# muzishen/IMAGDressing

Measured on AMD Instinct MI355X. Metric: 512x512 50-step images/sec (whole node), higher is better.
Workload: dtype bf16

## Files before the change

### imagdressing_amd/csrc/attention.hip

```cpp
#include "common.h"
#include "imd_kernels.h"

namespace {

constexpr int KT = 64;
constexpr int VSTR = KT * 2 + 16;

template <int D> struct AttnCfg {
    static constexpr int DPK = (D + 15) / 16 * 16;
    static constexpr int DPV = (D + 31) / 32 * 32;
    static constexpr int NKT = DPK / 16;
    static constexpr int NDT = DPV / 32;
    static constexpr int KSTR = DPK * 2 + 16;
    static constexpr int VROWS = DPV > D ? D + 1 : DPV;
    static constexpr int VBYTES = VROWS * VSTR;
    static constexpr int BUF = VBYTES + KT * KSTR;
    static_assert((DPV - VROWS) * VSTR <= KT * KSTR, "phantom V^T rows must stay inside the K tile");
    static constexpr int KVECS = (KT * (DPK / 8) + 255) / 256;
    static constexpr int VVECS = (D * (KT / 8) + 255) / 256;
};

typedef __attribute__((__vector_size__(4 * sizeof(uint32_t)))) uint32_t v4u;
__device__ __forceinline__ uint4 buf_load16(const __amdgpu_buffer_rsrc_t& rs, uint32_t byte_off) {
    const v4u v = __builtin_amdgcn_raw_buffer_load_b128(rs, (int)byte_off, 0, 0);
// ... 223 lines not shown
                for (int kb = 0; kb < KB; ++kb)
#pragma unroll
                    for (int r = 0; r < 16; ++r) mx = fmaxf(mx, s[qb][kb][r]);
                mx = fmaxf(mx, __shfl_xor(mx, 32));
                if (OFFS) {
                    if (first || __any(mx > OFFS_THR)) {
                        const float want = m_run[qb] + (first ? mx : fmaxf(mx, 0.f));
                        const float nref = E::tof(E::fromf(want));
                        const float delta = nref - m_run[qb];
                        if (!first) {
                            const float alpha = __builtin_amdgcn_exp2f(-delta);
#pragma unroll
                            for (int dt = 0; dt < C::NDT; ++dt)
#pragma unroll
                                for (int r = 0; r < 16; ++r) o[qb][dt][r] *= alpha;
                        }
#pragma unroll
                        for (int kb = 0; kb < KB; ++kb)
#pragma unroll
                            for (int r = 0; r < 16; ++r) s[qb][kb][r] -= delta;
                        m_run[qb] = nref;
                        if (hi == QPAD_HI) qf[qb][QPAD_T].x = (qf[qb][QPAD_T].x & 0xffff0000u) | (uint32_t)E::fromf(-nref);
                    }
#pragma unroll
                    for (int kb = 0; kb < KB; ++kb)
#pragma unroll
                        for (int r = 0; r < 16; ++r) s[qb][kb][r] = __builtin_amdgcn_exp2f(s[qb][kb][r]);
                } else {
                    const float m_new = fmaxf(m_run[qb], mx);
                    if (__any(m_new != m_run[qb])) {
                        const float alpha = __builtin_amdgcn_exp2f(m_run[qb] - m_new);
                        if (!LSUM_MFMA) l_run[qb] *= alpha;
#pragma unroll
                        for (int dt = 0; dt < C::NDT; ++dt)
#pragma unroll
                            for (int r = 0; r < 16; ++r) o[qb][dt][r] *= alpha;
                        m_run[qb] = m_new;
                    }
                    float psum = 0.f;
#pragma unroll
                    for (int kb = 0; kb < KB; ++kb)
#pragma unroll
                        for (int r = 0; r < 16; ++r) {
                            const float pe = __builtin_amdgcn_exp2f(s[qb][kb][r] - m_new);
                            s[qb][kb][r] = pe;
                            if (!LSUM_MFMA) psum += pe;
                        }
                    if (!LSUM_MFMA) l_run[qb] += psum;
                }
                pack_p();
            };
#pragma unroll
            for (int qb = 0; qb < QW; ++qb) {
                softmax_block(qb);
                if (PVSPLIT) {
#pragma unroll
                    for (int dt = 0; dt < C::NDT; ++dt)
#pragma unroll
                        for (int g = 0; g < 2 * KB; ++g) o[qb][dt] = E::mfma(vfr[dt][g], pf[qb][g], o[qb][dt]);
                        }
            }
            if (!PVSPLIT) {
#pragma unroll
                for (int dt = 0; dt < C::NDT; ++dt)
#pragma unroll
                    for (int g = 0; g < 2 * KB; ++g) {
                        const uint4 vf = *reinterpret_cast<const uint4*>(Vs + dt * 32 * VSTR + vfrag + (2 * k0 + g) * 32);
#pragma unroll
                        for (int qb = 0; qb < QW; ++qb) o[qb][dt] = E::mfma(vf, pf[qb][g], o[qb][dt]);
                    }
            }
            }
            if (t + 1 < ntiles) store_tile((t + 1) & 1);
            __syncthreads();
        }

#pragma unroll
        for (int qb = 0; qb < QW; ++qb) {
            float lt;
            if (LSUM_MFMA) {
                const float mine = o[qb][L_DT][L_REG];
                const float other = __shfl_xor(mine, 32);
                lt = (hi == L_HI) ? mine : other;
            } else {
                lt = l_run[qb] + __shfl_xor(l_run[qb], 32);
            }
            const float inv = ((ph == 1) ? w2 : 1.0f) / lt;
            const int q = q0 + qb * 32 + col;
            if (q >= p.N) continue;
            bf16_t* orow = p.out + ((size_t)b * p.N + q) * p.out_ld + h * D;
#pragma unroll
            for (int dt = 0; dt < C::NDT; ++dt)
#pragma unroll
                for (int j = 0; j < 4; ++j) {
                    const int dd = dt * 32 + 8 * j + 4 * hi;
                    if (dd >= D) continue;
                    float v[4];
#pragma unroll
                    for (int e = 0; e < 4; ++e) v[e] = o[qb][dt][4 * j + e] * inv;
                    if (second_only) {
                        *reinterpret_cast<float4*>(p.phase2_out + ((size_t)b * p.N + q) * (p.H * D) + h * D + dd) = make_float4(v[0], v[1], v[2], v[3]);
                        continue;
                    }
                    if (ph == 1) {
                        const uint2 prev = *reinterpret_cast<const uint2*>(orow + dd);
                        v[0] += E::lo(prev.x); v[1] += E::hi(prev.x); v[2] += E::lo(prev.y); v[3] += E::hi(prev.y);
                    }
                    *reinterpret_cast<uint2*>(orow + dd) = make_uint2(E::pack2(v[0], v[1]), E::pack2(v[2], v[3]));
                }
        }
    }
}

template <bool F16>
__global__ __launch_bounds__(256) void attn_phase_add_kernel(bf16_t* out, int out_ld, const float* __restrict__ add, int C, long rows) {
    using E = El<F16>;
    const int vpr = C / 4;
    const long total = rows * vpr;
    for (long i = blockIdx.x * 256L + threadIdx.x; i < total; i += (long)gridDim.x * 256L) {
        const long r = i / vpr;
        const int c = (int)(i - r * vpr) * 4;
        const float4 a = *reinterpret_cast<const float4*>(add + r * C + c);
        uint2* dst = reinterpret_cast<uint2*>(out + r * out_ld + c);
        const uint2 prev = *dst;
        *dst = make_uint2(E::pack2(a.x + E::lo(prev.x), a.y + E::hi(prev.x)), E::pack2(a.z + E::lo(prev.y), a.w + E::hi(prev.y)));
    }
}

template <bool F16, int D, int QW, int MINW, int KB = 2, bool SPEC = false, int SCHED = 0>
int launch_attn(const AttnParams& p, hipStream_t s) {
    using C = AttnCfg<D>;
    constexpr int lds = 2 * C::BUF;
    auto kern = attn_kernel<F16, D, QW, MINW, KB, SPEC, SCHED>;
    if (int rc_attr = imd_lds_attr(reinterpret_cast<const void*>(kern), lds, "attention")) return rc_attr;
    const int rows = 4 * QW * 32;
    dim3 grid((p.N + rows - 1) / rows, p.H, p.B + (p.phase2_rows > 0 ? p.phase2_rows : 0));
    hipLaunchKernelGGL(kern, grid, dim3(256), lds, s, p);
    int rc = imd_check_launch("attention");
    if (rc || p.phase2_rows <= 0) return rc;
    const long vecs = (long)p.phase2_rows * p.N * (p.H * D / 4);
    const int blocks = (int)((vecs + 255) / 256 < 4096 ? (vecs + 255) / 256 : 4096);
    hipLaunchKernelGGL(attn_phase_add_kernel<F16>, dim3(blocks), dim3(256), 0, s, p.out, p.out_ld, p.phase2_out, p.H * D, (long)p.phase2_rows * p.N);
    return imd_check_launch("attention (phase add)");
}

}

int g_attn_qw40 = 13;

int imd_attn_dpk(int D) { return (D + 15) / 16 * 16; }
int imd_attn_dpv(int D) { return (D + 31) / 32 * 32; }

int g_attn_xcd = 1;
#ifdef IMD_ATTN_SWEEP
int g_attn_v80 = 0, g_attn_v160 = 0;
#endif

int imd_attention_dup_supported(int H, int N, int D) { return (D == 40 && N >= 512 && H > 0) ? 1 : 0; }
int imd_attention_phase_split_supported(int D) { return (D == 64 || D == 80 || D == 160) ? 1 : 0; }

int imd_launch_attention(const AttnParams& p_in, hipStream_t s) {
    AttnParams p = p_in;
    const unsigned tag = (unsigned)p_in.flags & IMD_TUNING_TAG_MASK;
    if (tag != 0 && tag != (unsigned)IMD_TUNING_PER_CALL)
        return imd_set_error("attention: flags = 0x%x on entry is neither 0 nor IMD_TUNING_PER_CALL | bits (an uninitialised parameter block?)", (unsigned)p_in.flags);
    const bool per_call = tag == (unsigned)IMD_TUNING_PER_CALL;
    const int qw40 = (per_call && (p_in.flags & 255)) ? (p_in.flags & 255) : g_attn_qw40;
#ifdef IMD_ABLATIONS
    constexpr int QW40_MAX = 54;
#else
    constexpr int QW40_MAX = 13;
#endif
    if (qw40 < 1 || qw40 > QW40_MAX) return imd_set_error("attention: per-call head-dim-40 variant %d out of range 1..%d", qw40, QW40_MAX);
    p.flags = (per_call ? !((p_in.flags >> 8) & 1) : g_attn_xcd != 0) ? 0 : 1;
    if (p.B <= 0 || p.H <= 0 || p.N <= 0 || p.L1 <= 0) return imd_set_error("attention: empty problem B=%d H=%d N=%d L1=%d", p.B, p.H, p.N, p.L1);
    if (p.L1P % 64 || p.L1P < p.L1) return imd_set_error("attention: L1P (%d) must be a multiple of 64 and >= L1 (%d)", p.L1P, p.L1);
    if (p.k2 && (p.L2 <= 0 || p.L2P % 64 || p.L2P < p.L2)) return imd_set_error("attention: bad second key set L2=%d L2P=%d", p.L2, p.L2P);
    if (p.kv1_bdiv <= 0 || (p.k2 && p.kv2_bdiv <= 0)) return imd_set_error("attention: kv batch divisors must be positive");
    if (p.H > 65535 || p.B > 65535) return imd_set_error("attention: H/B exceed grid limits");
    if (p.dtype != IMD_DTYPE_BF16 && p.dtype != IMD_DTYPE_F16) return imd_set_error("attention: unknown dtype %d", p.dtype);
    if (p.causal && (p.k2 != nullptr || p.L1 != p.N)) return imd_set_error("attention: the causal mask needs a single key set with L1 == N");
    const bool h = p.dtype == IMD_DTYPE_F16;
    if ((p.phase2_rows != 0) != (p.phase2_out != nullptr)) return imd_set_error("attention: phase2_rows and phase2_out go together");
    if (p.phase2_rows != 0) {
        if (!imd_attention_phase_split_supported(p.D) || p.k2 == nullptr || p.scale2 == nullptr || p.causal || p.proj_w != nullptr || p.out_dup != nullptr ||
            p.phase2_rows < 0 || p.phase2_rows > p.B || (p.out_ld % 4) || p.B + p.phase2_rows > 65535)
            return imd_set_error("attention: phase2_rows needs head dim 64 / 80 / 160, a second key set with scale2, 0 < rows <= B, no causal mask / fused out-projection / "
                                 "out_dup (got D=%d rows=%d B=%d)", p.D, p.phase2_rows, p.B);
        if ((reinterpret_cast<uintptr_t>(p.phase2_out) & 15) || (reinterpret_cast<uintptr_t>(p.out) & 7))
            return imd_set_error("attention: phase2_out must be 16-byte aligned (out 8-byte)");
    }
    if (p.out_dup != nullptr) {
        if (!imd_attention_dup_supported(p.H, p.N, p.D) || !p.k_pad_one || p.causal || p.proj_w != nullptr)
            return imd_set_error("attention: out_dup needs head dim 40, N >= 512, k_pad_one, no causal mask and no fused out-projection (got D=%d N=%d k_pad_one=%d)", p.D, p.N, p.k_pad_one);
        if (p.out_dup == p.out) return imd_set_error("attention: out_dup must not alias out");
        return imd_launch_attention_d40(p, qw40 == 12 ? 12 : 13, s);
    }
    if (p.proj_w != nullptr) {
        if (p.D != 40 || p.H * p.D != 320 || p.N < 512 || p.causal)
            return imd_set_error("attention: the fused out-projection needs head dim 40, 8 heads, N >= 512, no causal mask (got D=%d H=%d N=%d)", p.D, p.H, p.N);
        if (!p.proj_out || !p.proj_counters) return imd_set_error("attention: fused out-projection without proj_out / proj_counters");
        if ((p.out_ld % 8) || (p.proj_out_ld % 8) || (p.proj_res && (p.proj_res_ld % 8)))
            return imd_set_error("attention: fused out-projection needs out_ld, proj_out_ld and proj_res_ld %% 8 == 0");
        if ((reinterpret_cast<uintptr_t>(p.out) | reinterpret_cast<uintptr_t>(p.proj_w) | reinterpret_cast<uintptr_t>(p.proj_out) |
             reinterpret_cast<uintptr_t>(p.proj_res) | reinterpret_cast<uintptr_t>(p.proj_b)) & 15)
            return imd_set_error("attention: fused out-projection needs 16-byte aligned out / proj_w / proj_out / proj_res / proj_b");
        if ((size_t)p.B * p.N * p.out_ld * 2 >= 0x80000000ull) return imd_set_error("attention: fused out-projection: out buffer beyond 2 GiB");
        return imd_launch_attention_d40(p, 10, s);
    }
    switch (p.D) {
        case 40:
            if (qw40 >= 6 && p.N >= 512 && !p.causal) return imd_launch_attention_d40(p, qw40, s);
            if (qw40 == 2 && p.N >= 512) return h ? launch_attn<true, 40, 2, 2, 1, true, 1>(p, s) : launch_attn<false, 40, 2, 2, 1, true, 1>(p, s);
            if (qw40 == 5 && p.N >= 512) return h ? launch_attn<true, 40, 2, 2, 1, true, 3>(p, s) : launch_attn<false, 40, 2, 2, 1, true, 3>(p, s);
            if (qw40 == 3) return h ? launch_attn<true, 40, 1, 3, 2, false>(p, s) : launch_attn<false, 40, 1, 3, 2, false>(p, s);
            if (qw40 == 4) return h ? launch_attn<true, 40, 1, 3, 1, true>(p, s) : launch_attn<false, 40, 1, 3, 1, true>(p, s);
            if (qw40 == 1 && p.N >= 512) return h ? launch_attn<true, 40, 2, 2, 1, true, 0>(p, s) : launch_attn<false, 40, 2, 2, 1, true, 0>(p, s);
            return h ? launch_attn<true, 40, 1, 3, 1, true>(p, s) : launch_attn<false, 40, 1, 3, 1, true>(p, s);
        case 64: return h ? launch_attn<true, 64, 1, 2>(p, s) : launch_attn<false, 64, 1, 2>(p, s);
        case 80:
#ifdef IMD_ATTN_SWEEP
            switch (g_attn_v80) {
                case 1: return h ? launch_attn<true, 80, 1, 2, 2, false, 0>(p, s) : launch_attn<false, 80, 1, 2, 2, false, 0>(p, s);
                case 2: return h ? launch_attn<true, 80, 1, 3, 1, false, 0>(p, s) : launch_attn<false, 80, 1, 3, 1, false, 0>(p, s);
                case 3: return h ? launch_attn<true, 80, 1, 3, 1, false, 2>(p, s) : launch_attn<false, 80, 1, 3, 1, false, 2>(p, s);
                case 4: return h ? launch_attn<true, 80, 2, 1, 2, false, 0>(p, s) : launch_attn<false, 80, 2, 1, 2, false, 0>(p, s);
                case 5: return h ? launch_attn<true, 80, 2, 1, 2, false, 3>(p, s) : launch_attn<false, 80, 2, 1, 2, false, 3>(p, s);
                case 6: return h ? launch_attn<true, 80, 2, 1, 1, false, 3>(p, s) : launch_attn<false, 80, 2, 1, 1, false, 3>(p, s);
                case 7: return h ? launch_attn<true, 80, 1, 2, 1, false, 2>(p, s) : launch_attn<false, 80, 1, 2, 1, false, 2>(p, s);
                default: break;
            }
#endif
            return h ? launch_attn<true, 80, 1, 2, 2, false, 2>(p, s) : launch_attn<false, 80, 1, 2, 2, false, 2>(p, s);
        case 160:
#ifdef IMD_ATTN_SWEEP
            switch (g_attn_v160) {
                case 1: return h ? launch_attn<true, 160, 1, 1, 2, false, 0>(p, s) : launch_attn<false, 160, 1, 1, 2, false, 0>(p, s);
                case 2: return h ? launch_attn<true, 160, 1, 1, 1, false, 2>(p, s) : launch_attn<false, 160, 1, 1, 1, false, 2>(p, s);
                case 3: return h ? launch_attn<true, 160, 1, 2, 1, false, 0>(p, s) : launch_attn<false, 160, 1, 2, 1, false, 0>(p, s);
                default: break;
            }
#endif
            return h ? launch_attn<true, 160, 1, 1, 2, false, 2>(p, s) : launch_attn<false, 160, 1, 1, 2, false, 2>(p, s);
        default: return imd_set_error("attention: unsupported head dim %d (supported: 40, 64, 80, 160)", p.D);
    }
}
```

### imagdressing_amd/csrc/capi.cpp

```cpp
#include <atomic>
#include <mutex>
#include <stdarg.h>
#include <stdio.h>
#include <string.h>

#include "imd_kernels.h"

namespace {
thread_local char g_err[512] = "";
}

int imd_set_error(const char* fmt, ...) {
    va_list ap;
    va_start(ap, fmt);
    vsnprintf(g_err, sizeof(g_err), fmt, ap);
    va_end(ap);
    return 1;
}

int imd_check_launch(const char* what) {
    hipError_t e = hipGetLastError();
    if (e != hipSuccess) return imd_set_error("%s: launch failed: %s", what, hipGetErrorString(e));
    return 0;
}

#define IMD_REQUIRE(cond, ...) do { if (!(cond)) return imd_set_error(__VA_ARGS__); } while (0)
#define IMD_REQUIRE_SIZE(p, what) IMD_REQUIRE((p)->struct_bytes == sizeof(*(p)), \
    "%s: parameter block is %u bytes in the caller's view, this library (ABI v%d) expects %zu: the binding mirrors another version of include/imagdressing_hip.h (set struct_bytes = sizeof(struct) after zero-initialising it)", \
    what, (unsigned)(p)->struct_bytes, IMD_ABI_VERSION, sizeof(*(p)))

namespace {
struct LdsAttrEnt { const void* kern; int dev; };
constexpr int kMaxLdsAttr = 512;
LdsAttrEnt g_lds_attr[kMaxLdsAttr];
std::atomic<int> g_lds_attr_n{0};
std::mutex g_lds_attr_mu;
int g_cu8[64] = {};
}

int imd_lds_attr(const void* kern, int bytes, const char* what) {
    int dev = 0;
    if (hipGetDevice(&dev) != hipSuccess) return imd_set_error("%s: cannot identify the current device", what);
    const int n = g_lds_attr_n.load(std::memory_order_acquire);
    for (int i = 0; i < n; ++i)
        if (g_lds_attr[i].kern == kern && g_lds_attr[i].dev == dev) return 0;
    std::lock_guard<std::mutex> lock(g_lds_attr_mu);
    hipError_t e = hipFuncSetAttribute(kern, hipFuncAttributeMaxDynamicSharedMemorySize, bytes);
    if (e != hipSuccess) return imd_set_error("%s: hipFuncSetAttribute failed: %s", what, hipGetErrorString(e));
    const int m = g_lds_attr_n.load(std::memory_order_relaxed);
    if (m < kMaxLdsAttr) {
        g_lds_attr[m] = LdsAttrEnt{kern, dev};
        g_lds_attr_n.store(m + 1, std::memory_order_release);
    }
    return 0;
}

int imd_cu_count8() {
    int dev = 0;
    if (hipGetDevice(&dev) != hipSuccess || dev < 0 || dev >= 64) return -1;
    if (g_cu8[dev] == 0) {
        int cus = 0;
        if (hipDeviceGetAttribute(&cus, hipDeviceAttributeMultiprocessorCount, dev) != hipSuccess) return -1;
        g_cu8[dev] = cus / 8 * 8 < 8 ? 8 : cus / 8 * 8;
    }
    return g_cu8[dev];
}

extern "C" {

int imd_abi_version(void) { return IMD_ABI_VERSION; }
const char* imd_last_error(void) { return g_err; }

int imd_device_check(int device) {
    hipDeviceProp_t prop;
    hipError_t e = hipGetDeviceProperties(&prop, device);
    if (e != hipSuccess) return imd_set_error("device_check: hipGetDeviceProperties(%d) failed: %s", device, hipGetErrorString(e));
    if (strncmp(prop.gcnArchName, "gfx950", 6) != 0)
        return imd_set_error("device_check: device %d is %s; this library is built for gfx950 (MI355X) only", device, prop.gcnArchName);
    return 0;
}

int imd_conv_gemm(const imd_conv_gemm_params* p, int cfg, void* stream) {
    IMD_REQUIRE(p != nullptr, "conv_gemm: null params");
    IMD_REQUIRE_SIZE(p, "conv_gemm");
    IMD_REQUIRE(p->x && p->w, "conv_gemm: null input/weight pointer");
    IMD_REQUIRE(p->mode == IMD_OUT_HEADS || p->out != nullptr, "conv_gemm: null output pointer");
    IMD_REQUIRE(p->Hout > 0 && p->Wout > 0 && p->Hin > 0 && p->Win > 0, "conv_gemm: bad geometry");
    IMD_REQUIRE(p->stride == 1 || p->stride == 2, "conv_gemm: stride must be 1 or 2");
    IMD_REQUIRE(p->M % (p->Hout * p->Wout) == 0, "conv_gemm: M (%d) is not a multiple of Hout*Wout (%d)", p->M, p->Hout * p->Wout);
    if (p->mode == IMD_OUT_HEADS) {
        IMD_REQUIRE(p->hC > 0 && p->hH > 0 && p->hD > 0 && p->hC == p->hH * p->hD, "conv_gemm: bad head split C=%d H=%d D=%d", p->hC, p->hH, p->hD);
        IMD_REQUIRE(p->N % p->hC == 0 && p->N / p->hC <= 3, "conv_gemm: N (%d) must be 1..3 splits of %d channels", p->N, p->hC);
        IMD_REQUIRE(p->hD % 8 == 0, "conv_gemm: head dim must be a multiple of 8");
        IMD_REQUIRE(p->act != IMD_ACT_GEGLU && !p->out_f32, "conv_gemm: head-split output excludes GEGLU / fp32 output");
    }
    if (p->act == IMD_ACT_GEGLU) IMD_REQUIRE(!p->out_f32 && !p->res, "conv_gemm: GEGLU excludes fp32 output and residual");
    return imd_launch_conv_gemm(*p, cfg, (hipStream_t)stream);
}

int imd_conv_gemm_auto_cfg(int M, int N) { return imd_conv_gemm_choose_cfg(M, N); }
int imd_conv_gemm_auto_split(int M, int N, int K, int cfg) { return imd_conv_gemm_choose_split(M, N, K, cfg < 0 ? imd_conv_gemm_choose_cfg(M, N) : cfg); }

int imd_attention(const imd_attn_params* p, void* stream) {
    IMD_REQUIRE(p != nullptr, "attention: null params");
    IMD_REQUIRE_SIZE(p, "attention");
    IMD_REQUIRE(p->q && p->k1 && p->v1t && p->out, "attention: null q/k/v/out pointer");
    IMD_REQUIRE((p->k2 == nullptr) == (p->v2t == nullptr), "attention: k2 and v2t must be given together");
    IMD_REQUIRE(p->out_ld >= p->H * p->D && p->out_ld % 4 == 0, "attention: bad out_ld %d", p->out_ld);
    return imd_launch_attention(*p, (hipStream_t)stream);
}

int imd_attention_fp8(const imd_attn_params* p, int eq, int ek, int ev, void* stream) {
    IMD_REQUIRE(p != nullptr, "attention_fp8: null params");
    IMD_REQUIRE_SIZE(p, "attention_fp8");
    IMD_REQUIRE(p->q && p->k1 && p->v1t && p->out, "attention_fp8: null q/k/v/out pointer");
    IMD_REQUIRE((p->k2 == nullptr) == (p->v2t == nullptr), "attention_fp8: k2 and v2t must be given together");
    IMD_REQUIRE(p->out_ld >= p->H * p->D && p->out_ld % 4 == 0, "attention_fp8: bad out_ld %d", p->out_ld);
    IMD_REQUIRE(p->dtype == IMD_DTYPE_BF16 || p->dtype == IMD_DTYPE_F16, "attention_fp8: unknown output dtype %d", p->dtype);
    return imd_launch_attention_fp8(*p, eq, ek, ev, (hipStream_t)stream);
}

int imd_attn_quantize_fp8(const uint16_t* src, uint8_t* dst, int kind, long count, int LP, int exp2_scale, float pad_val, int dtype,
                          void* stream) {
    IMD_REQUIRE(src && dst && count > 0, "attn_quantize_fp8: null pointer / empty");
    IMD_REQUIRE(kind == 0 || kind == 1, "attn_quantize_fp8: kind must be 0 (Q / K rows) or 1 (V^T)");
    IMD_REQUIRE(exp2_scale >= -16 && exp2_scale <= 16, "attn_quantize_fp8: exponent out of range");
    return imd_launch_attn_quantize_fp8(src, dst, kind, count, LP, exp2_scale, pad_val, dtype, (hipStream_t)stream);
}

int imd_set_tuning(int knob, int value) {
    switch (knob) {
        case 0:
#ifdef IMD_ABLATIONS
            IMD_REQUIRE(value >= 1 && value <= 54, "set_tuning: attention variant for head dim 40 must be 1..54 (20..49: timing ablations, WRONG results; 50..54: correct but no faster)");
#else
            IMD_REQUIRE(value >= 1 && value <= 13, "set_tuning: attention variant for head dim 40 must be 1..13 (the timing ablations 20..49 and the measured no-gain variants 50..54 exist only in -DIMD_ABLATIONS builds)");
#endif
            g_attn_qw40 = value; return 0;
        case 1: g_attn_xcd = value ? 1 : 0; return 0;
        case 2:
#ifndef IMD_ABLATIONS
            IMD_REQUIRE((value & 224) == 0, "set_tuning: bits 5..7 of knob 2 are the timing ablations of gemm_dma256.hip (WRONG results); they exist only in -DIMD_ABLATIONS builds");
#endif
            IMD_REQUIRE((value & ~2047) == 0, "set_tuning: knob 2 has bits 0..10 only (got %d)", value);
            g_gemm_flags = value; return 0;
#ifdef IMD_ATTN_SWEEP
        case 3: g_attn_v80 = value; return 0;
        case 4: g_attn_v160 = value; return 0;
#endif
        default: return imd_set_error("set_tuning: unknown knob %d", knob);
    }
}

int imd_get_tuning(int knob) { return knob == 0 ? g_attn_qw40 : knob == 1 ? g_attn_xcd : knob == 2 ? g_gemm_flags : -1; }

int imd_attn_padded_dims(int D, int* dpk, int* dpv) {
    IMD_REQUIRE(D == 40 || D == 64 || D == 80 || D == 160, "attn_padded_dims: unsupported head dim %d", D);
    if (dpk) *dpk = imd_attn_dpk(D);
    if (dpv) *dpv = imd_attn_dpv(D);
    return 0;
}

int imd_groupnorm(const imd_groupnorm_params* p, void* stream) {
    IMD_REQUIRE(p != nullptr, "groupnorm: null params");
    IMD_REQUIRE_SIZE(p, "groupnorm");
    IMD_REQUIRE(p->x && p->y && p->gamma && p->beta && p->partial, "groupnorm: null pointer");
    return imd_launch_groupnorm(*p, (hipStream_t)stream);
}

int imd_groupnorm_coeffs(const imd_groupnorm_params* p, float* coef_a, float* coef_b, void* stream) {
    IMD_REQUIRE(p != nullptr, "groupnorm_coeffs: null params");
    IMD_REQUIRE_SIZE(p, "groupnorm_coeffs");
    IMD_REQUIRE(p->x && p->gamma && p->beta && p->partial && coef_a && coef_b, "groupnorm_coeffs: null pointer");
    return imd_launch_groupnorm_coeffs(*p, coef_a, coef_b, (hipStream_t)stream);
}

static bool sized(const imd_conv_gemm_params* p) { return p && p->struct_bytes == sizeof(*p); }
static int query(const imd_conv_gemm_params* p, bool (*pred)(const imd_conv_gemm_params&)) {
    if (!sized(p)) return 0;
    imd_conv_gemm_params q = *p;
    if (!imd_conv_gemm_fill_extents(q)) return 0;
    return pred(q) ? 1 : 0;
}
int imd_conv_patch_supported(const imd_conv_gemm_params* p) { return query(p, static_cast<bool (*)(const imd_conv_gemm_params&)>(imd_conv_patch_supported)); }
int imd_conv_patch2_supported(const imd_conv_gemm_params* p) { return query(p, static_cast<bool (*)(const imd_conv_gemm_params&)>(imd_conv_patch2_supported)); }
int imd_conv_patch3_supported(const imd_conv_gemm_params* p) { return query(p, static_cast<bool (*)(const imd_conv_gemm_params&)>(imd_conv_patch3_supported)); }
int imd_conv_patch4_supported(const imd_conv_gemm_params* p) { return query(p, static_cast<bool (*)(const imd_conv_gemm_params&)>(imd_conv_patch4_supported)); }
int imd_conv_img_supported(const imd_conv_gemm_params* p) { return query(p, static_cast<bool (*)(const imd_conv_gemm_params&)>(imd_conv_img_supported)); }
int imd_conv_patch_stats_parts(const imd_conv_gemm_params* p) { return sized(p) ? imd_conv_patch_stats_parts_of(*p) : 0; }
int imd_conv_gemm_stats_parts(const imd_conv_gemm_params* p, int cfg) { return sized(p) ? imd_conv_gemm_stats_parts_of(*p, cfg) : 0; }
int imd_row_linear_gn_in_supported(const imd_conv_gemm_params* p, int cfg) { return (sized(p) && p->gn_in_partial != nullptr && imd_row_linear_gn_in_supported_of(*p, cfg)) ? 1 : 0; }
int imd_conv_gemm_gn_out_supported(const imd_conv_gemm_params* p) { return (sized(p) && imd_conv_gemm_gn_out_supported_of(*p, -1)) ? 1 : 0; }
int imd_gemm_dma_supported(const imd_conv_gemm_params* p) { return query(p, static_cast<bool (*)(const imd_conv_gemm_params&)>(imd_gemm_dma_supported)); }

int imd_row_linear_supported(const imd_conv_gemm_params* p) { return (sized(p) && (imd_row_linear_supported(*p) || imd_row_linear_k640_supported(*p) || imd_row_linear_k1280_supported(*p) || imd_row_qkv_supported(*p))) ? 1 : 0; }

int imd_row_linear(const imd_conv_gemm_params* p, int ln, float ln_eps, void* stream) {
    IMD_REQUIRE(p != nullptr, "row_linear: null params");
    IMD_REQUIRE_SIZE(p, "row_linear");
    IMD_REQUIRE(p->x && p->w, "row_linear: null input/weight pointer");
    IMD_REQUIRE(p->mode == IMD_OUT_HEADS || p->out != nullptr, "row_linear: null output pointer");
    IMD_REQUIRE(p->Hout > 0 && p->Wout > 0 && p->M > 0 && p->M % (p->Hout * p->Wout) == 0, "row_linear: bad geometry");
    if (p->mode == IMD_OUT_HEADS) {
        IMD_REQUIRE(p->hC > 0 && p->hH > 0 && p->hD > 0 && p->hC == p->hH * p->hD && p->N % p->hC == 0 && p->N / p->hC <= 3 && p->hD % 8 == 0,
                    "row_linear: bad head split C=%d H=%d D=%d", p->hC, p->hH, p->hD);
        IMD_REQUIRE(!p->out_f32, "row_linear: head-split output excludes fp32 output");
    }
    IMD_REQUIRE(!ln || ln_eps > 0.f, "row_linear: LayerNorm needs eps > 0");
    if (p->K == 320 && p->N == 960 && p->mode == IMD_OUT_HEADS) {
        IMD_REQUIRE(p->gn_in_partial == nullptr, "row_linear: the fused q / k / v projection has no GroupNorm prologue (gn_in_*)");
        return imd_launch_row_qkv(*p, ln, ln_eps, (hipStream_t)stream);
    }
    if (p->K == 640) return imd_launch_row_linear_k640(*p, ln, ln_eps, (hipStream_t)stream);
    if (p->K == 1280) return imd_launch_row_linear_k1280(*p, ln, ln_eps, (hipStream_t)stream);
    return imd_launch_row_linear(*p, ln, ln_eps, (hipStream_t)stream);
}

int imd_ff_geglu(const imd_ff_params* p, void* stream) {
    IMD_REQUIRE(p != nullptr, "ff_geglu: null params");
    IMD_REQUIRE_SIZE(p, "ff_geglu");
    IMD_REQUIRE(p->x && p->w1 && p->b1 && p->w2 && p->b2 && p->out, "ff_geglu: null pointer");
    IMD_REQUIRE(!p->ln || p->ln_eps > 0.f, "ff_geglu: LayerNorm needs eps > 0");
    return imd_launch_ff_geglu(*p, (hipStream_t)stream);
}

int imd_layernorm(const imd_layernorm_params* p, void* stream) {
    IMD_REQUIRE(p != nullptr, "layernorm: null params");
    IMD_REQUIRE_SIZE(p, "layernorm");
    IMD_REQUIRE(p->x && p->y && p->gamma && p->beta, "layernorm: null pointer");
    return imd_launch_layernorm(*p, (hipStream_t)stream);
}

int imd_embed_tokens(const uint16_t* table, int vocab, const uint16_t* pos, int T, const int64_t* ids, uint16_t* out, long rows, int C,
                     int dtype, void* stream) {
    IMD_REQUIRE(table && pos && ids && out, "embed_tokens: null pointer");
    return imd_launch_embed_tokens(table, vocab, pos, T, ids, out, rows, C, dtype, (hipStream_t)stream);
}

int imd_vit_assemble(const uint16_t* patches, const uint16_t* cls, const uint16_t* pos, uint16_t* out, int B, int P, int C, int dtype,
                     void* stream) {
    IMD_REQUIRE(patches && cls && pos && out, "vit_assemble: null pointer");
    return imd_launch_vit_assemble(patches, cls, pos, out, B, P, C, dtype, (hipStream_t)stream);
}

int imd_lincomb(const float* const* xs, const float* coefs, int n, float* out, long numel, void* stream) {
    IMD_REQUIRE(xs && coefs && out, "lincomb: null pointer");
    return imd_launch_lincomb(xs, coefs, n, out, numel, (hipStream_t)stream);
}

int imd_softmax_rows(const float* s, int s_ld, uint16_t* p, int p_ld, int rows, int cols, int dtype, void* stream) {
    IMD_REQUIRE(s && p, "softmax_rows: null pointer");
    return imd_launch_softmax_rows(s, s_ld, p, p_ld, rows, cols, dtype, (hipStream_t)stream);
}

int imd_ddim_cfg_step(const imd_ddim_params* p, void* stream) {
    IMD_REQUIRE(p != nullptr, "ddim_cfg_step: null params");
    IMD_REQUIRE_SIZE(p, "ddim_cfg_step");
    IMD_REQUIRE(p->z && p->eps, "ddim_cfg_step: null pointer");
    IMD_REQUIRE(p->coefs != nullptr || p->sqrt_a_t > 0.f, "ddim_cfg_step: sqrt(alpha_t) must be positive");
    return imd_launch_ddim_cfg_step(*p, (hipStream_t)stream);
}

int imd_ddim_cfg_step_rows(const imd_ddim_params* p, const float* guidance, void* stream) {
    IMD_REQUIRE(p != nullptr, "ddim_cfg_step_rows: null params");
    IMD_REQUIRE_SIZE(p, "ddim_cfg_step_rows");
    IMD_REQUIRE(p->z && p->eps && guidance, "ddim_cfg_step_rows: null pointer");
    IMD_REQUIRE(p->coefs != nullptr || p->sqrt_a_t > 0.f, "ddim_cfg_step_rows: sqrt(alpha_t) must be positive");
    return imd_launch_ddim_cfg_step_rows(*p, guidance, (hipStream_t)stream);
}

int imd_timestep_embedding(const float* t, float* out, int B, int dim, void* stream) {
    IMD_REQUIRE(t && out, "timestep_embedding: null pointer");
    return imd_launch_timestep_embedding(t, out, B, dim, (hipStream_t)stream);
}

int imd_add(const uint16_t* a, int a_ld, const uint16_t* b, int b_ld, uint16_t* out, int out_ld, long rows, int C, float b_scale, int dtype, void* stream) {
    IMD_REQUIRE(a && b && out, "add: null pointer");
    return imd_launch_add(a, a_ld, b, b_ld, out, out_ld, rows, C, b_scale, dtype, (hipStream_t)stream);
}

int imd_copy2d(const uint16_t* a, int a_ld, uint16_t* out, int out_ld, long rows, int C, void* stream) {
    IMD_REQUIRE(a && out, "copy2d: null pointer");
    return imd_launch_copy2d(a, a_ld, out, out_ld, rows, C, (hipStream_t)stream);
}

int imd_concat2(const uint16_t* a, int Ca, const uint16_t* b, int Cb, const uint16_t* b_add, uint16_t* out, long rows, long b_rows, int dtype, void* stream) {
    IMD_REQUIRE(a && b && out, "concat2: null pointer");
    return imd_launch_concat2(a, Ca, b, Cb, b_add, out, rows, b_rows, dtype, (hipStream_t)stream);
}

int imd_groupnorm_parts(int B, int HW, int C) { return imd_groupnorm_parts_of(B, HW, C); }

int imd_concat2_gn_stats(const uint16_t* a, int Ca, const uint16_t* b, int Cb, const uint16_t* b_add, uint16_t* out, int B, int HW, int b_B, int G,
                         float* partial, int dtype, void* stream) {
    IMD_REQUIRE(a && b && out && partial, "concat2 + statistics: null pointer");
    return imd_launch_concat2_gn_stats(a, Ca, b, Cb, b_add, out, B, HW, b_B, G, partial, dtype, (hipStream_t)stream);
}

int imd_f32_to_16(const float* a, uint16_t* out, long n, int dtype, void* stream) {
    IMD_REQUIRE(a && out, "f32_to_16: null pointer");
// ... 5 lines not shown
```

### imagdressing_amd/csrc/imd_kernels.h

```cpp
#pragma once
#include <hip/hip_runtime.h>
#include <stdint.h>

#include "../../include/imagdressing_hip.h"

typedef uint16_t bf16_t;
typedef imd_heads_dest HeadsDest;
typedef imd_conv_gemm_params ConvGemmParams;
typedef imd_attn_params AttnParams;
typedef imd_groupnorm_params GroupNormParams;
typedef imd_layernorm_params LayerNormParams;
typedef imd_ddim_params DdimParams;

enum { ACT_NONE = IMD_ACT_NONE, ACT_SILU = IMD_ACT_SILU, ACT_GEGLU = IMD_ACT_GEGLU, ACT_GELU = IMD_ACT_GELU, ACT_QUICK_GELU = IMD_ACT_QUICK_GELU };
enum { OUT_ROWMAJOR = IMD_OUT_ROWMAJOR, OUT_HEADS = IMD_OUT_HEADS };

int imd_set_error(const char* fmt, ...);
int imd_check_launch(const char* what);
int imd_lds_attr(const void* kern, int bytes, const char* what);
int imd_cu_count8();

int imd_conv_gemm_choose_cfg(int M, int N);
int imd_conv_gemm_choose_split(int M, int N, int K, int cfg);
int imd_launch_conv_gemm(const ConvGemmParams& p, int cfg, hipStream_t s);
bool imd_conv_gemm_fill_extents(ConvGemmParams& p);
bool imd_conv_patch_supported(const ConvGemmParams& p);
bool imd_conv_patch2_supported(const ConvGemmParams& p);
int imd_launch_conv_patch2(const ConvGemmParams& p, hipStream_t s);
bool imd_conv_patch3_supported(const ConvGemmParams& p);
int imd_launch_conv_patch3(const ConvGemmParams& p, hipStream_t s);
bool imd_conv_patch4_supported(const ConvGemmParams& p);
int imd_launch_conv_patch4(const ConvGemmParams& p, hipStream_t s);
int imd_conv_patch3_stats_parts_of(const ConvGemmParams& p, int nw);
bool imd_conv_patch64_supported(const ConvGemmParams& p);
int imd_launch_conv_patch64(const ConvGemmParams& p, hipStream_t s);
bool imd_conv_img_supported(const ConvGemmParams& p);
int imd_launch_conv_img(const ConvGemmParams& p, hipStream_t s);
int imd_conv_patch_stats_parts_of(const ConvGemmParams& p);
int imd_conv_gemm_stats_parts_of(const ConvGemmParams& p, int cfg);
bool imd_conv_gemm_gn_out_supported_of(const ConvGemmParams& p, int cfg);
bool imd_row_linear_gn_in_supported_of(const ConvGemmParams& p, int cfg);
int imd_launch_conv_patch(const ConvGemmParams& p, hipStream_t s);
bool imd_row_linear_supported(const ConvGemmParams& p);
int imd_launch_row_linear(const ConvGemmParams& p, int ln, float ln_eps, hipStream_t s);
bool imd_row_linear_k640_supported(const ConvGemmParams& p);
int imd_launch_row_linear_k640(const ConvGemmParams& p, int ln, float ln_eps, hipStream_t s);
bool imd_row_linear_k1280_supported(const ConvGemmParams& p);
int imd_launch_row_linear_k1280(const ConvGemmParams& p, int ln, float ln_eps, hipStream_t s);
bool imd_row_qkv_supported(const ConvGemmParams& p);
int imd_launch_row_qkv(const ConvGemmParams& p, int ln, float ln_eps, hipStream_t s);
bool imd_gemm_dma_supported(const ConvGemmParams& p);
int imd_launch_gemm_dma(const ConvGemmParams& p, hipStream_t s);
int imd_launch_gemm_dma128(const ConvGemmParams& p, int stages, hipStream_t s);
int imd_launch_gemm_dma256(const ConvGemmParams& p, int form, hipStream_t s);
bool imd_conv_dma_supported(const ConvGemmParams& p);
int imd_launch_ff_geglu(const imd_ff_params& p, hipStream_t s);
int imd_launch_attention(const AttnParams& p, hipStream_t s);
int imd_launch_attention_d40(const AttnParams& p, int variant, hipStream_t s);
int imd_launch_attention_fp8(const AttnParams& p, int eq, int ek, int ev, hipStream_t s);
int imd_launch_attn_quantize_fp8(const bf16_t* src, unsigned char* dst, int kind, long rows_or_groups, int LP, int exp2_scale,
                                 float pad_val, int dtype, hipStream_t s);
extern int g_attn_qw40;
extern int g_attn_xcd;
#ifdef IMD_ATTN_SWEEP
extern int g_attn_v80, g_attn_v160;
#endif
extern int g_gemm_flags;
int imd_attn_dpk(int D);
int imd_attn_dpv(int D);
int imd_launch_groupnorm(const GroupNormParams& p, hipStream_t s);
int imd_launch_groupnorm_coeffs(const GroupNormParams& p, float* ca, float* cb, hipStream_t s);
int imd_groupnorm_parts_of(int B, int HW, int C);
int imd_launch_concat2_gn_stats(const bf16_t* a, int Ca, const bf16_t* b, int Cb, const bf16_t* b_add, bf16_t* out, int B, int HW, int b_B, int G,
                                float* partial, int dtype, hipStream_t s);
int imd_launch_layernorm(const LayerNormParams& p, hipStream_t s);
int imd_launch_softmax_rows(const float* s_in, int s_ld, bf16_t* p_out, int p_ld, int rows, int cols, int dtype, hipStream_t s);
int imd_launch_ddim_cfg_step(const DdimParams& p, hipStream_t s);
int imd_launch_ddim_cfg_step_rows(const DdimParams& p, const float* guidance, hipStream_t s);
int imd_launch_timestep_embedding(const float* t, float* out, int B, int dim, hipStream_t s);
int imd_launch_add(const bf16_t* a, int a_ld, const bf16_t* b, int b_ld, bf16_t* out, int out_ld, long rows, int C, float b_scale, int dtype, hipStream_t s);
int imd_launch_embed_tokens(const bf16_t* table, int vocab, const bf16_t* pos, int T, const int64_t* ids, bf16_t* out, long rows, int C, int dtype, hipStream_t s);
int imd_launch_vit_assemble(const bf16_t* patches, const bf16_t* cls, const bf16_t* pos, bf16_t* out, int B, int P, int C, int dtype, hipStream_t s);
int imd_launch_lincomb(const float* const* xs, const float* coefs, int n, float* out, long numel, hipStream_t s);
int imd_launch_copy2d(const bf16_t* a, int a_ld, bf16_t* out, int out_ld, long rows, int C, hipStream_t s);
int imd_launch_concat2(const bf16_t* a, int Ca, const bf16_t* b, int Cb, const bf16_t* b_add, bf16_t* out, long rows, long b_rows, int dtype, hipStream_t s);
int imd_launch_f32_to_16(const float* a, bf16_t* out, long n, int dtype, hipStream_t s);
```

Measured before the change: 6.957.

## Add dedicated head-dim-80 attention kernel with LDS DMA ring pipeline

Adds a specialised flash-attention kernel for head dimension 80. It streams K and V^T tiles into a three-slot LDS ring using buffer-to-LDS DMA, and software-pipelines the fragment loads, MFMAs and softmax work across two 32-key steps. It also uses a lazy max-offset rescaling that only rescales when the running max grows past a threshold. The kernel is dispatched by default for non-causal, single-phase calls with N>=512 and L1>128, replacing the generic templated path there. This adds a large new code path with XCD-aware block remapping, at the cost of more complexity and a risk of numerical or edge-case differences.

Measured after the change: 6.978, median of 6. No clear change (+0.3%).

```diff
diff --git a/imagdressing_amd/csrc/attention.hip b/imagdressing_amd/csrc/attention.hip
--- a/imagdressing_amd/csrc/attention.hip
+++ b/imagdressing_amd/csrc/attention.hip
@@ -399,8 +399,10 @@
 int imd_attn_dpv(int D) { return (D + 31) / 32 * 32; }
 
 int g_attn_xcd = 1;
+int g_attn_v80 = 0;
+constexpr int ATTN80_MIN_N = 512, ATTN80_MIN_L1 = 128;
 #ifdef IMD_ATTN_SWEEP
-int g_attn_v80 = 0, g_attn_v160 = 0;
+int g_attn_v160 = 0;
 #endif
 
 int imd_attention_dup_supported(int H, int N, int D) { return (D == 40 && N >= 512 && H > 0) ? 1 : 0; }
@@ -466,10 +468,18 @@
             return h ? launch_attn<true, 40, 1, 3, 1, true>(p, s) : launch_attn<false, 40, 1, 3, 1, true>(p, s);
         case 64: return h ? launch_attn<true, 64, 1, 2>(p, s) : launch_attn<false, 64, 1, 2>(p, s);
         case 80:
+            if (!p.causal && p.phase2_rows == 0 && (g_attn_v80 == 2 || (p.N >= ATTN80_MIN_N && p.L1 > ATTN80_MIN_L1))) {
+                if (g_attn_v80 == 0 || g_attn_v80 == 2) return imd_launch_attention_d80(p, 0, s);
+#ifdef IMD_ATTN_SWEEP
+                if (g_attn_v80 == 9) return imd_launch_attention_d80(p, 9, s);
+#endif
+#ifdef IMD_ABLATIONS
+                if (g_attn_v80 >= 20) return imd_launch_attention_d80(p, g_attn_v80, s);
+#endif
+            }
 #ifdef IMD_ATTN_SWEEP
             switch (g_attn_v80) {
                 case 1: return h ? launch_attn<true, 80, 1, 2, 2, false, 0>(p, s) : launch_attn<false, 80, 1, 2, 2, false, 0>(p, s);
-                case 2: return h ? launch_attn<true, 80, 1, 3, 1, false, 0>(p, s) : launch_attn<false, 80, 1, 3, 1, false, 0>(p, s);
                 case 3: return h ? launch_attn<true, 80, 1, 3, 1, false, 2>(p, s) : launch_attn<false, 80, 1, 3, 1, false, 2>(p, s);
                 case 4: return h ? launch_attn<true, 80, 2, 1, 2, false, 0>(p, s) : launch_attn<false, 80, 2, 1, 2, false, 0>(p, s);
                 case 5: return h ? launch_attn<true, 80, 2, 1, 2, false, 3>(p, s) : launch_attn<false, 80, 2, 1, 2, false, 3>(p, s);
diff --git a/imagdressing_amd/csrc/attention_d80.hip b/imagdressing_amd/csrc/attention_d80.hip
--- /dev/null
+++ b/imagdressing_amd/csrc/attention_d80.hip
@@ -0,0 +1,323 @@
+#include <type_traits>
+#include "lds_dma.h"
+
+#include "common.h"
+#include "imd_kernels.h"
+
+namespace {
+
+constexpr int D = 80, DPK = 80, DPV = 96, NKT = DPK / 16, NDT = DPV / 32;
+constexpr int KT = 64;
+constexpr int KSTR = DPK * 2, VSTR = KT * 2;
+constexpr int VROWS = D + 1;
+constexpr int VBYTES = VROWS * VSTR;
+constexpr int KBYTES = KT * KSTR;
+constexpr int BUF = VBYTES + KBYTES;
+static_assert((DPV - VROWS) * VSTR <= KBYTES, "phantom V^T rows must stay inside the K rows");
+constexpr int NRING = 3;
+constexpr int NKP = KBYTES / 1024, NVP = D * VSTR / 1024, NPIECE = (NKP + NVP) / 4;
+static_assert(NKP * 1024 == KBYTES && NVP * 1024 == D * VSTR && NPIECE * 4 == NKP + NVP, "a unit is a whole number of pieces per wave");
+constexpr int NF = NKT + 2 * NDT;
+constexpr uint32_t OOB = 0xffffffffu;
+constexpr int QW_SHIP = 1;
+
+template <bool F16, int QW, int VAR>
+__global__ __launch_bounds__(256, QW == 1 ? 2 : 1) void attn80_kernel(const AttnParams p) {
+    using E = El<F16>;
+    constexpr int L_DT = D / 32, L_REG = ((D % 32) & 3) + 4 * ((D % 32) >> 3), L_HI = ((D % 32) >> 2) & 1;
+    constexpr int PD = QW == 1 ? 3 : 2;
+    constexpr int NFR = PD + 1;
+    constexpr int NM = NF * QW;
+    constexpr float OFFS_THR = 8.0f;
+    extern __shared__ __attribute__((aligned(16))) char smem[];
+
+    const int tid = threadIdx.x;
+    const int lane = tid & 63;
+    const int wave = tid >> 6;
+    const int hi = lane >> 5;
+    const int col = lane & 31;
+    int wx, h, b;
+    {
+        const unsigned gx = gridDim.x, gy = gridDim.y, gz = gridDim.z, total = gx * gy * gz;
+        const unsigned Lb = blockIdx.x + gx * (blockIdx.y + gy * blockIdx.z);
+        const unsigned xcd = Lb & 7u, slot = Lb >> 3;
+        const unsigned q8 = total >> 3, r8 = total & 7u;
+        unsigned w = (xcd < r8 ? xcd * (q8 + 1) : r8 * (q8 + 1) + (xcd - r8) * q8) + slot;
+        if (p.flags & 1) w = Lb;
+        wx = (int)(w % gx);
+        b = (int)((w / gx) % gz);
+        h = (int)(w / (gx * gz));
+    }
+    const int q0 = (wx * 4 + wave) * (QW * 32);
+
+    {
+        const uint32_t one2 = E::pack2(1.0f, 1.0f);
+        for (int v = tid; v < NRING * (VSTR / 16); v += 256)
+            *reinterpret_cast<uint4*>(smem + (v / (VSTR / 16)) * BUF + D * VSTR + (v % (VSTR / 16)) * 16) = make_uint4(one2, one2, one2, one2);
+    }
+
+    uint4 qf[QW][NKT];
+#pragma unroll
+    for (int qb = 0; qb < QW; ++qb) {
+        const int q = q0 + qb * 32 + col;
+#pragma unroll
+        for (int t = 0; t < NKT; ++t) {
+            uint4 v = make_uint4(0, 0, 0, 0);
+            if (q < p.N) v = *reinterpret_cast<const uint4*>(p.q + ((size_t)(b * p.H + h) * p.N + q) * DPK + t * 16 + hi * 8);
+            qf[qb][t] = v;
+        }
+    }
+
+    float w2 = 0.f;
+    if (p.k2 != nullptr && p.scale2 != nullptr) w2 = p.scale2[b];
+    const int nph = (w2 != 0.f) ? 2 : 1;
+
+    const int kfd = swap23(col) * KSTR + ((hi ^ ((col >> 2) & 1)) << 4);
+    int vfd[4];
+#pragma unroll
+    for (int g = 0; g < 4; ++g) vfd[g] = col * VSTR + (((2 * g + hi) ^ ((col >> 1) & 7)) << 4);
+    const f32x16 zero16 = {0.f, 0.f, 0.f, 0.f, 0.f, 0.f, 0.f, 0.f, 0.f, 0.f, 0.f, 0.f, 0.f, 0.f, 0.f, 0.f};
+    const int wv = __builtin_amdgcn_readfirstlane(wave);
+    const uint32_t smem_base = (uint32_t)(uintptr_t)smem;
+
+    for (int ph = 0; ph < nph; ++ph) {
+        f32x16 o[QW][NDT];
+        float m_ref[QW];
+        f32x16 cinit[QW];
+#pragma unroll
+        for (int qb = 0; qb < QW; ++qb) {
+            m_ref[qb] = 0.f;
+            cinit[qb] = zero16;
+#pragma unroll
+            for (int dt = 0; dt < NDT; ++dt) o[qb][dt] = zero16;
+        }
+        const int L = ph ? p.L2 : p.L1;
+        const int LP = ph ? p.L2P : p.L1P;
+        const int kvb = ph ? (b / p.kv2_bdiv) : (b / p.kv1_bdiv);
+        const bf16_t* kbase = (ph ? p.k2 : p.k1) + (size_t)(kvb * p.H + h) * L * DPK;
+        const bf16_t* vbase = (ph ? p.v2t : p.v1t) + (size_t)(kvb * p.H + h) * DPV * LP;
+        const int J = (L + 31) >> 5;
+        const int NU = (J >> 1) + 1;
+
+        const v4i_t ds_k = raw_rsrc(kbase, (uint32_t)L * DPK * 2), ds_v = raw_rsrc(vbase, (uint32_t)D * LP * 2);
+        int dsrc[NPIECE];
+        bool dneg[NPIECE];
+#pragma unroll
+        for (int i = 0; i < NPIECE; ++i) {
+            const int qi = wv + 4 * i;
+            if (qi < NKP) {
+                const int sl = 64 * qi + lane, r = sl / 10, c = (sl % 10) ^ ((r >> 3) & 1);
+                dsrc[i] = (32 + r) * KSTR + c * 16;
+                dneg[i] = r < 32;
+            } else {
+                const int sl = 64 * (qi - NKP) + lane, dd = sl >> 3, c = (sl & 7) ^ ((dd >> 1) & 7);
+                dsrc[i] = (dd * LP + c * 8 - 32) * 2;
+                dneg[i] = c < 4;
+            }
+        }
+        auto dma_piece = [&](int u, int bufi, int i, auto loop_c) __attribute__((always_inline)) {
+            constexpr bool LOOP = decltype(loop_c)::value;
+            const int qi = wv + 4 * i;
+            const bool isk = qi < NKP;
+            const bool bad = !LOOP && (isk ? (u < 0 && dneg[i]) : (u <= 0 && (u < 0 || dneg[i])));
+            const uint32_t off = bad ? OOB : (uint32_t)(dsrc[i] + u * (isk ? KBYTES : KT * 2));
+            const uint32_t dst = smem_base + bufi * BUF + (isk ? VBYTES + 1024 * qi : 1024 * (qi - NKP));
+            if (LOOP) dma16_nonop(isk ? ds_k : ds_v, dst, off);
+            else dma16(isk ? ds_k : ds_v, dst, off);
+        };
+        auto dma_unit = [&](int u, int bufi, auto loop_c) __attribute__((always_inline)) {
+#pragma unroll
+            for (int i = 0; i < NPIECE; ++i) dma_piece(u, bufi, i, loop_c);
+        };
+
+        f32x16 sa[QW], sb[QW];
+        uint4 pa[QW][2], pb[QW][2];
+#pragma unroll
+        for (int qb = 0; qb < QW; ++qb)
+#pragma unroll
+            for (int g = 0; g < 2; ++g) pb[qb][g] = make_uint4(0, 0, 0, 0);
+        uint4 fr[NFR];
+
+        auto step = [&](const char* Vs, auto second_c, int j, f32x16 (&sc)[QW], f32x16 (&sn)[QW], uint4 (&pc)[QW][2], uint4 (&pp)[QW][2]) __attribute__((always_inline)) {
+            constexpr bool SECOND = decltype(second_c)::value;
+            constexpr int KB = SECOND ? 1 : 0, G0 = SECOND ? 2 : 0, R0 = SECOND ? (NF % NFR) : 0;
+            const char* Ks = Vs + VBYTES;
+            if (j * 32 + 32 > L) {
+#pragma unroll
+                for (int qb = 0; qb < QW; ++qb)
+#pragma unroll
+                    for (int r = 0; r < 16; ++r) {
+                        const int key = j * 32 + 8 * hi + (r & 7) + 16 * (r >> 3);
+                        if (key >= L) sc[qb][r] = -INFINITY;
+                    }
+            }
+            auto frag = [&](int f, int kb, int g0) -> uint4 {
+                if ((VAR & 1024) && f > 0) f = 0;
+                return f < NKT ? *reinterpret_cast<const uint4*>(Ks + kb * 32 * KSTR + kfd + f * 32)
+                               : *reinterpret_cast<const uint4*>(Vs + ((f - NKT) >> 1) * 32 * VSTR + vfd[g0 + ((f - NKT) & 1)]);
+            };
+            auto mma = [&](int i, const uint4& fa) {
+                const int f = i / QW, qb = i % QW;
+                if (f < NKT) { if (!(VAR & 64) || f == 0) sn[qb] = E::mfma(fa, qf[qb][f], f == 0 ? cinit[qb] : sn[qb]); }
+                else if (!(VAR & 32)) o[qb][(f - NKT) >> 1] = E::mfma(fa, pp[qb][(f - NKT) & 1], o[qb][(f - NKT) >> 1]);
+            };
+            float dlt[QW];
+#pragma unroll
+            for (int qb = 0; qb < QW; ++qb) dlt[qb] = 0.f;
+            bool fix = false;
+            auto word = [&](int qb, int w) -> uint32_t& {
+                uint4& v = pc[qb][w >> 2];
+                return (w & 3) == 0 ? v.x : (w & 3) == 1 ? v.y : (w & 3) == 2 ? v.z : v.w;
+            };
+            auto vwork = [&](int qb, int k) {
+                if (k == 0) {
+                    float mx = __builtin_fmaxf(__builtin_fmaxf(sc[qb][0], sc[qb][1]), sc[qb][2]);
+#pragma unroll
+                    for (int r = 3; r < 15; r += 2) mx = __builtin_fmaxf(__builtin_fmaxf(mx, sc[qb][r]), sc[qb][r + 1]);
+                    mx = __builtin_fmaxf(mx, sc[qb][15]);
+                    const auto sw = __builtin_amdgcn_permlane32_swap(__float_as_uint(mx), __float_as_uint(mx), false, false);
+                    mx = __builtin_fmaxf(__uint_as_float(sw[0]), __uint_as_float(sw[1]));
+                    const bool first = j == 0;
+                    if (__builtin_expect(first || __any(mx > OFFS_THR), 0)) {
+                        const float d = first ? mx : __builtin_fmaxf(mx, 0.f);
+#pragma unroll
+                        for (int r = 0; r < 16; ++r) sc[qb][r] -= d;
+                        m_ref[qb] += d;
+#pragma unroll
+                        for (int r = 0; r < 16; ++r) cinit[qb][r] = -m_ref[qb];
+                        dlt[qb] = d;
+                        fix = true;
+                    }
+                    return;
+                }
+                if (k <= 8 && !(VAR & 4)) {
+                    const int r0 = 2 * (k - 1);
+                    sc[qb][r0] = __builtin_amdgcn_exp2f(sc[qb][r0]);
+                    sc[qb][r0 + 1] = __builtin_amdgcn_exp2f(sc[qb][r0 + 1]);
+                }
+                if (k >= 2 && k <= 9) {
+                    uint32_t& w = word(qb, k - 2);
+                    w = E::pack2(sc[qb][2 * (k - 2)], sc[qb][2 * (k - 2) + 1]);
+                    asm volatile("" : "+v"(w));
+                }
+            };
+            if (!SECOND) {
+#pragma unroll
+                for (int f = 0; f < PD; ++f) fr[f] = frag(f, KB, G0);
+            }
+            __builtin_amdgcn_sched_barrier(0);
+#pragma unroll
+            for (int i = 0; i < NM; ++i) {
+                if (i % QW == 0) {
+                    const int f2 = i / QW + PD;
+                    if (f2 < NF) fr[(R0 + f2) % NFR] = frag(f2, KB, G0);
+                    else if (!SECOND) fr[(R0 + f2) % NFR] = frag(f2 - NF, 1, 2);
+                }
+                mma(i, fr[(R0 + i / QW) % NFR]);
+                vwork(i / NF, i % NF);
+                __builtin_amdgcn_sched_barrier(0);
+            }
+            if (fix) {
+#pragma unroll
+                for (int qb = 0; qb < QW; ++qb) {
+#pragma unroll
+                    for (int r = 0; r < 16; ++r) sn[qb][r] -= dlt[qb];
+                    if (j != 0) {
+                        const float alpha = __builtin_amdgcn_exp2f(-dlt[qb]);
+#pragma unroll
+                        for (int dt = 0; dt < NDT; ++dt)
+#pragma unroll
+                            for (int r = 0; r < 16; ++r) o[qb][dt][r] *= alpha;
+                    }
+                }
+            }
+        };
+
+        dma_unit(-1, 2, std::false_type{});
+        dma_unit(0, 0, std::false_type{});
+        dma_unit(1, 1, std::false_type{});
+        dma_wait();
+        __syncthreads();
+        {
+            const char* Ks = smem + 2 * BUF + VBYTES + 32 * KSTR;
+#pragma unroll
+            for (int tk = 0; tk < NKT; ++tk) {
+                const uint4 kf = *reinterpret_cast<const uint4*>(Ks + kfd + tk * 32);
+#pragma unroll
+                for (int qb = 0; qb < QW; ++qb) sa[qb] = E::mfma(kf, qf[qb][tk], tk == 0 ? zero16 : sa[qb]);
+            }
+        }
+        __syncthreads();
+
+        int ring = 0;
+        for (int u = 0; u < NU; ++u) {
+            const int dbuf = ring == 0 ? 2 : ring - 1;
+            if (!(VAR & 16)) dma_unit(u + 2, dbuf, std::true_type{});
+            const char* Vs = smem + ring * BUF;
+            ring = ring == NRING - 1 ? 0 : ring + 1;
+            step(Vs, std::false_type{}, 2 * u, sa, sb, pa, pb);
+            step(Vs, std::true_type{}, 2 * u + 1, sb, sa, pb, pa);
+            dma_wait_keep_n<NPIECE>();
+            if (!(VAR & 8)) __syncthreads();
+        }
+        dma_wait();
+        __syncthreads();
+
+#pragma unroll
+        for (int qb = 0; qb < QW; ++qb) {
+            const float mine = o[qb][L_DT][L_REG];
+            const float other = __shfl_xor(mine, 32);
+            const float lt = (hi == L_HI) ? mine : other;
+            const float inv = ((ph == 1) ? w2 : 1.0f) / lt;
+            const int q = q0 + qb * 32 + col;
+            if (q >= p.N) continue;
+            bf16_t* orow = p.out + ((size_t)b * p.N + q) * p.out_ld + h * D;
+            uint2 prev[D / 8];
+            if (ph == 1) {
+#pragma unroll
+                for (int jj = 0; jj < D / 8; ++jj) prev[jj] = *reinterpret_cast<const uint2*>(orow + 8 * jj + 4 * hi);
+            }
+#pragma unroll
+            for (int jq = 0; jq < D / 8; ++jq) {
+                const int dt = jq >> 2, jj = jq & 3;
+                float v[4];
+#pragma unroll
+                for (int e = 0; e < 4; ++e) v[e] = o[qb][dt][4 * jj + e] * inv;
+                if (ph == 1) { v[0] += E::lo(prev[jq].x); v[1] += E::hi(prev[jq].x); v[2] += E::lo(prev[jq].y); v[3] += E::hi(prev[jq].y); }
+                prev[jq] = make_uint2(E::pack2(v[0], v[1]), E::pack2(v[2], v[3]));
+            }
+#pragma unroll
+            for (int jq = 0; jq < D / 8; ++jq) *reinterpret_cast<uint2*>(orow + 8 * jq + 4 * hi) = prev[jq];
+        }
+    }
+}
+
+template <bool F16, int QW, int VAR>
+int launch_attn80(const AttnParams& p, hipStream_t s) {
+    auto kern = attn80_kernel<F16, QW, VAR>;
+    constexpr int LDS_BYTES = NRING * BUF;
+    if (int rc_attr = imd_lds_attr(reinterpret_cast<const void*>(kern), LDS_BYTES, "attention(d=80)")) return rc_attr;
+    dim3 grid((p.N + 128 * QW - 1) / (128 * QW), p.H, p.B);
+    hipLaunchKernelGGL(kern, grid, dim3(256), LDS_BYTES, s, p);
+    return imd_check_launch("attention(d=80)");
+}
+
+}
+
+int imd_launch_attention_d80(const AttnParams& p, int variant, hipStream_t s) {
+    const bool h = p.dtype == IMD_DTYPE_F16;
+    switch (variant) {
+#ifdef IMD_ATTN_SWEEP
+        case 9: return h ? launch_attn80<true, 3 - QW_SHIP, 0>(p, s) : launch_attn80<false, 3 - QW_SHIP, 0>(p, s);
+#endif
+#ifdef IMD_ABLATIONS
+        case 20: return launch_attn80<false, QW_SHIP, 4>(p, s);
+        case 21: return launch_attn80<false, QW_SHIP, 8>(p, s);
+        case 22: return launch_attn80<false, QW_SHIP, 8 | 16>(p, s);
+        case 23: return launch_attn80<false, QW_SHIP, 32>(p, s);
+        case 24: return launch_attn80<false, QW_SHIP, 64>(p, s);
+        case 25: return launch_attn80<false, QW_SHIP, 1024>(p, s);
+#endif
+        default: return h ? launch_attn80<true, QW_SHIP, 0>(p, s) : launch_attn80<false, QW_SHIP, 0>(p, s);
+    }
+}
diff --git a/imagdressing_amd/csrc/capi.cpp b/imagdressing_amd/csrc/capi.cpp
--- a/imagdressing_amd/csrc/capi.cpp
+++ b/imagdressing_amd/csrc/capi.cpp
@@ -144,8 +144,8 @@
 #endif
             IMD_REQUIRE((value & ~2047) == 0, "set_tuning: knob 2 has bits 0..10 only (got %d)", value);
             g_gemm_flags = value; return 0;
+        case 3: g_attn_v80 = value; return 0;
 #ifdef IMD_ATTN_SWEEP
-        case 3: g_attn_v80 = value; return 0;
         case 4: g_attn_v160 = value; return 0;
 #endif
         default: return imd_set_error("set_tuning: unknown knob %d", knob);
diff --git a/imagdressing_amd/csrc/imd_kernels.h b/imagdressing_amd/csrc/imd_kernels.h
--- a/imagdressing_amd/csrc/imd_kernels.h
+++ b/imagdressing_amd/csrc/imd_kernels.h
@@ -62,8 +62,10 @@
                                  float pad_val, int dtype, hipStream_t s);
 extern int g_attn_qw40;
 extern int g_attn_xcd;
+int imd_launch_attention_d80(const AttnParams& p, int variant, hipStream_t s);
+extern int g_attn_v80;
 #ifdef IMD_ATTN_SWEEP
-extern int g_attn_v80, g_attn_v160;
+extern int g_attn_v160;
 #endif
 extern int g_gemm_flags;
 int imd_attn_dpk(int D);
```
